# instadeepai/FrameDiPT

Hardware: AMD Instinct MI355X
Metric: residue*diffusion-steps/sec (higher is better)
Workload: dtype fp16

## Files before the change

### framedipt_amd/csrc/rowblock.hip

```cpp
#include <type_traits>

#include "common.hpp"
#include "kernels.hpp"

#pragma clang fp contract(off)

#define RB_SROW 144

typedef fd_h rb_hx4 __attribute__((ext_vector_type(4)));
__device__ __forceinline__ hx8 rb_ld(const char* p) { return __builtin_bit_cast(hx8, *(const u16x8*)p); }
__host__ __device__ constexpr int rb_max(int a, int b) { return a > b ? a : b; }

template <int N, class F>
__device__ __forceinline__ void ch_rb_for(F&& f) {
  if constexpr (N > 0) {
    ch_rb_for<N - 1>(f);
    f(std::integral_constant<int, N - 1>{});
  }
}

template <int K0, int N1, int N2, int NOUT, int FLAGS>
struct RBShape {
  static constexpr int KS0 = (K0 + 15) / 16;
  static constexpr int NL = 1 + (N1 > 0) + (N2 > 0);
// ... 413 lines not shown
    w_load(std::integral_constant<int, 0>{}, (const char*)img, wave);
    if constexpr (SPLIT) w_load(std::integral_constant<int, 1>{}, (const char*)img_lo, wave);
  };
  auto put4 = [&](char* buf, int off, float v0, float v1, float v2, float v3) {
    const float v[4] = {v0, v1, v2, v3};
    rb_hx4 pk, pl;
#pragma unroll
    for (int q = 0; q < 4; ++q) {
      pk[q] = (fd_h)v[q];
      pl[q] = (fd_h)(v[q] - (float)pk[q]);
    }
    *(rb_hx4*)(buf + off) = pk;
    if constexpr (SPLIT) *(rb_hx4*)(buf + XLO + off) = pl;
  };
  w_first(a.wo, a.wol);
  {
    f32x4 xv[10];
#pragma unroll
    for (int k = 0; k < 10; ++k) {
      const int idx = tid + k * FD_THREADS, r = idx / 80, c4 = idx % 80;
      const int gr = row0 + r < a.M ? row0 + r : a.M - 1;
      xv[k] = *(const f32x4*)(a.att + (long)gr * a.ld + 4 * c4);
    }
    {
      constexpr int NC = 7 * TL_D + (POST ? TL_NP : 0), NCV = (NC + FD_THREADS - 1) / FD_THREADS;
      float cv[NCV];
#pragma unroll
      for (int k = 0; k < NCV; ++k) {
        const int v = tid + k * FD_THREADS, which = v / TL_D, c = v % TL_D;
        const float* src = which == 0 ? a.bo : which == 1 ? a.g1 : which == 2 ? a.be1 : which == 3 ? a.b1 : which == 4 ? a.b2 : which == 5 ? a.g2 : a.be2;
        cv[k] = v < 7 * TL_D ? src[c] : (POST && v < NC ? a.bp[v - 7 * TL_D] : 0.f);
      }
#pragma unroll
      for (int k = 0; k < NCV; ++k)
        if (tid + k * FD_THREADS < NC) cst[tid + k * FD_THREADS] = cv[k];
    }
#pragma unroll
    for (int k = 0; k < 10; ++k) {
      const int idx = tid + k * FD_THREADS, r = idx / 80, c4 = idx % 80;
      put4(xs, r * TL_XROW + 8 * c4, xv[k][0], xv[k][1], xv[k][2], xv[k][3]);
    }
  }
  f32x4 rv[3][4];
#pragma unroll
  for (int u = 0; u < 3; ++u)
#pragma unroll
    for (int it = 0; it < 4; ++it) {
      const int T = wave + 4 * u < TL_NT ? wave + 4 * u : wave;
      const int r = 8 * it + (lane >> 3), gr = row0 + r < a.M ? row0 + r : a.M - 1;
      rv[u][it] = *(const f32x4*)(a.x + (long)gr * a.ld + 32 * T + 4 * (lane & 7));
    }
  f32x4 rvp[POST ? 2 : 1][4];
  auto load_rvp = [&]() {
#pragma unroll
    for (int u = 0; u < (POST ? 2 : 0); ++u)
#pragma unroll
      for (int it = 0; it < 4; ++it) {
        const int r = 8 * it + (lane >> 3), gr = row0 + r < a.M ? row0 + r : a.M - 1;
        rvp[u][it] = *(const f32x4*)(a.pres + (long)gr * a.ld_pres + 32 * (wave + 4 * u) + 4 * (lane & 7));
      }
  };
  if constexpr (POST && !SPLIT) load_rvp();
  const unsigned warm_tok = fd_l2_warm(a.warm, blockIdx.x, gridDim.x, tid, FD_THREADS);
  __syncthreads();
  FD_STAMP(1);
  hx8 X[TL_KS];
  f32x16 acc[3], xa[3];
  const char* xl_base = nullptr;
  auto x_load = [&](const char* buf) {
#pragma unroll
    for (int s = 0; s < TL_KS; ++s) X[s] = rb_ld(buf + li * TL_XROW + 32 * s + 16 * hi);
    xl_base = buf + XLO + li * TL_XROW + 16 * hi;
  };
  auto layer = [&](const void* img_, const void* img_lo_, auto NTC) {
    constexpr int NT = decltype(NTC)::value, NU = (NT + 3) / 4;
    const char* img = (const char*)img_;
    const char* img_lo = (const char*)img_lo_;
    ch_rb_for<NU>([&](auto U) {
      constexpr int u = decltype(U)::value;
      const int T = wave + 4 * u;
      const bool more = u + 1 < NU && T + 4 < NT;
      if constexpr (SPLIT) {
        constexpr int HB = (2 * u) % 3, LB = (2 * u + 1) % 3, FB = (2 * u + 2) % 3;
        if (more) w_load(std::integral_constant<int, FB>{}, img, T + 4);
        if (T < NT) {
          f32x16 c;
#pragma unroll
          for (int r = 0; r < 16; ++r) c[r] = 0.f;
#pragma unroll
          for (int s = 0; s < TL_KS; ++s) c = fd_mfma32(Wf[HB][s], X[s], c);
          {
            hx8 xr[3];
            xr[0] = rb_ld(xl_base);
            xr[1] = rb_ld(xl_base + 32);
            __builtin_amdgcn_sched_barrier(0);
#pragma unroll
            for (int s = 0; s < TL_KS; ++s) {
              if (s + 2 < TL_KS) xr[(s + 2) % 3] = rb_ld(xl_base + 32 * (s + 2));
              c = fd_mfma32(Wf[HB][s], xr[s % 3], c);
              __builtin_amdgcn_sched_barrier(0);
            }
          }
          if (more) w_load(std::integral_constant<int, HB>{}, img_lo, T + 4);
#pragma unroll
          for (int s = 0; s < TL_KS; ++s) c = fd_mfma32(Wf[LB][s], X[s], c);
          acc[u] = c;
        }
      } else {
        if (more) {
          if (u & 1) w_load(std::integral_constant<int, 0>{}, img, T + 4);
          else w_load(std::integral_constant<int, 1>{}, img, T + 4);
        }
        if (T < NT) {
          f32x16 c;
#pragma unroll
          for (int r = 0; r < 16; ++r) c[r] = 0.f;
#pragma unroll
          for (int s = 0; s < TL_KS; ++s) c = fd_mfma32(Wf[u & 1][s], X[s], c);
          acc[u] = c;
        }
      }
    });
  };
  constexpr std::integral_constant<int, TL_NT> NT_D{};
  auto layernorm = [&](const float* gam, const float* bet) {
    float s1 = 0.f, s2 = 0.f;
#pragma unroll
    for (int u = 0; u < 3; ++u)
      if (wave + 4 * u < TL_NT)
#pragma unroll
        for (int r = 0; r < 16; ++r) {
          s1 += acc[u][r];
          s2 += acc[u][r] * acc[u][r];
        }
    s1 += __shfl_xor(s1, 32, 64);
    s2 += __shfl_xor(s2, 32, 64);
    __syncthreads();
    if (hi == 0) {
      red[0][wave][li] = s1;
      red[1][wave][li] = s2;
    }
    __syncthreads();
    const float mu = (red[0][0][li] + red[0][1][li] + red[0][2][li] + red[0][3][li]) * (1.0f / TL_D);
    const float ex2 = (red[1][0][li] + red[1][1][li] + red[1][2][li] + red[1][3][li]) * (1.0f / TL_D);
    const float rstd = 1.0f / sqrtf(fmaxf(ex2 - mu * mu, 0.f) + 1e-5f);
#pragma unroll
    for (int u = 0; u < 3; ++u) {
      const int T = wave + 4 * u;
      if (T < TL_NT)
#pragma unroll
        for (int g = 0; g < 4; ++g) {
          const int f0 = 32 * T + 8 * g + 4 * hi;
          const f32x4 gm = *(const f32x4*)(gam + f0), bt = *(const f32x4*)(bet + f0);
#pragma unroll
          for (int q = 0; q < 4; ++q) acc[u][4 * g + q] = (acc[u][4 * g + q] - mu) * rstd * gm[q] + bt[q];
        }
    }
  };
  x_load(xs);
  layer(a.wo, a.wol, NT_D);
  FD_STAMP(2);
  w_first(a.w1, a.w1l);
#pragma unroll
  for (int u = 0; u < 3; ++u) {
    const int T = wave + 4 * u;
    if (T < TL_NT) {
#pragma unroll
      for (int it = 0; it < 4; ++it) *(f32x4*)(stg + (8 * it + (lane >> 3)) * RB_SROW + 16 * (lane & 7)) = rv[u][it];
#pragma unroll
      for (int g = 0; g < 4; ++g) {
        const f32x4 bv = *(const f32x4*)(cst + 32 * T + 8 * g + 4 * hi);
        const f32x4 rr = *(const f32x4*)(stg + li * RB_SROW + (8 * g + 4 * hi) * 4);
#pragma unroll
        for (int q = 0; q < 4; ++q) acc[u][4 * g + q] += bv[q] + rr[q];
      }
    }
  }
  layernorm(cst + TL_D, cst + 2 * TL_D);
  FD_STAMP(3);
#pragma unroll
  for (int u = 0; u < 3; ++u) {
    const int T = wave + 4 * u;
    xa[u] = acc[u];
    if (T < TL_NT)
#pragma unroll
      for (int g = 0; g < 4; ++g) {
        const int f0 = 32 * T + 8 * g + 4 * hi;
        put4(hs, li * TL_XROW + 2 * f0, acc[u][4 * g], acc[u][4 * g + 1], acc[u][4 * g + 2], acc[u][4 * g + 3]);
      }
  }
  __syncthreads();
  x_load(hs);
  FD_STAMP(4);
  layer(a.w1, a.w1l, NT_D);
  FD_STAMP(5);
  w_first(a.w2, a.w2l);
#pragma unroll
  for (int u = 0; u < 3; ++u) {
    const int T = wave + 4 * u;
    if (T < TL_NT)
#pragma unroll
      for (int g = 0; g < 4; ++g) {
        const int f0 = 32 * T + 8 * g + 4 * hi;
        const f32x4 bv = *(const f32x4*)(cst + 3 * TL_D + f0);
        put4(xs, li * TL_XROW + 2 * f0, fmaxf(acc[u][4 * g] + bv[0], 0.f), fmaxf(acc[u][4 * g + 1] + bv[1], 0.f),
             fmaxf(acc[u][4 * g + 2] + bv[2], 0.f), fmaxf(acc[u][4 * g + 3] + bv[3], 0.f));
      }
  }
  __syncthreads();
  x_load(xs);
  FD_STAMP(6);
  layer(a.w2, a.w2l, NT_D);
  FD_STAMP(7);
#pragma unroll
  for (int u = 0; u < 3; ++u) {
    const int T = wave + 4 * u;
    if (T < TL_NT)
#pragma unroll
      for (int g = 0; g < 4; ++g) {
        const f32x4 bv = *(const f32x4*)(cst + 4 * TL_D + 32 * T + 8 * g + 4 * hi);
#pragma unroll
        for (int q = 0; q < 4; ++q) acc[u][4 * g + q] += bv[q] + xa[u][4 * g + q];
      }
  }
  if constexpr (POST && SPLIT) load_rvp();
  if constexpr (POST) w_first(a.wp, a.wpl);
  layernorm(cst + 5 * TL_D, cst + 6 * TL_D);
  FD_STAMP(8);
  if constexpr (POST) {
#pragma unroll
    for (int u = 0; u < 3; ++u) {
      const int T = wave + 4 * u;
      if (T < TL_NT)
#pragma unroll
        for (int g = 0; g < 4; ++g) {
          const int f0 = 32 * T + 8 * g + 4 * hi;
          put4(hs, li * TL_XROW + 2 * f0, acc[u][4 * g], acc[u][4 * g + 1], acc[u][4 * g + 2], acc[u][4 * g + 3]);
        }
    }
    __syncthreads();
    x_load(hs);
    layer(a.wp, a.wpl, std::integral_constant<int, TL_NP / 32>{});
#pragma unroll
    for (int u = 0; u < 2; ++u) {
      const int T = wave + 4 * u;
#pragma unroll
      for (int it = 0; it < 4; ++it) *(f32x4*)(stg + (8 * it + (lane >> 3)) * RB_SROW + 16 * (lane & 7)) = rvp[u][it];
#pragma unroll
      for (int g = 0; g < 4; ++g) {
        const f32x4 bv = *(const f32x4*)(cst + 7 * TL_D + 32 * T + 8 * g + 4 * hi);
        const f32x4 rr = *(const f32x4*)(stg + li * RB_SROW + (8 * g + 4 * hi) * 4);
        f32x4 o;
#pragma unroll
        for (int q = 0; q < 4; ++q) o[q] = acc[u][4 * g + q] + bv[q] + rr[q];
        *(f32x4*)(stg + li * RB_SROW + (8 * g + 4 * hi) * 4) = o;
      }
#pragma unroll
      for (int it = 0; it < 4; ++it) {
        const int r = 8 * it + (lane >> 3);
        const f32x4 o = *(const f32x4*)(stg + r * RB_SROW + 16 * (lane & 7));
        if (row0 + r < a.M) *(f32x4*)(a.pout + (long)(row0 + r) * a.ld_pout + 32 * T + 4 * (lane & 7)) = o;
      }
    }
    fd_l2_warm_done(warm_tok);
    return;
  }
#pragma unroll
  for (int u = 0; u < 3; ++u) {
    const int T = wave + 4 * u;
    if (T < TL_NT) {
#pragma unroll
      for (int g = 0; g < 4; ++g) {
        f32x4 o = {acc[u][4 * g], acc[u][4 * g + 1], acc[u][4 * g + 2], acc[u][4 * g + 3]};
        *(f32x4*)(stg + li * RB_SROW + (8 * g + 4 * hi) * 4) = o;
      }
#pragma unroll
      for (int it = 0; it < 4; ++it) {
        const int r = 8 * it + (lane >> 3);
        const f32x4 o = *(const f32x4*)(stg + r * RB_SROW + 16 * (lane & 7));
        if (row0 + r < a.M) *(f32x4*)(a.out + (long)(row0 + r) * a.ld + 32 * T + 4 * (lane & 7)) = o;
      }
    }
  }
  fd_l2_warm_done(warm_tok);
}

#define RB16_BLOCKS 1
#define T16_KS (TL_D / 32)
#define T16_NT (TL_D / 16)
#define T16_XROW (TL_D * 2 + 32)
#define T16_XLO (16 * T16_XROW)
#define T16_SMEM (4 * T16_XLO + (7 * TL_D + TL_NP) * 4 + 2 * 4 * 16 * 4 + 16)
template <bool POST>
__global__ __launch_bounds__(FD_THREADS, RB16_BLOCKS) void tfmr_tail16_kernel(TfmrTailArgs a) {
  extern __shared__ __attribute__((aligned(16))) char smem[];
  char* xs = smem;
  char* hs = xs + 2 * T16_XLO;
  float* cst = (float*)(hs + 2 * T16_XLO);
  float (*red)[4][16] = (float (*)[4][16])(cst + 7 * TL_D + TL_NP);
  const int tid = threadIdx.x, lane = tid & 63, wave = tid >> 6, lr = lane & 15, fg = lane >> 4;
  const int row0 = blockIdx.x * 16;
  const long grow = row0 + lr < a.M ? row0 + lr : a.M - 1;
  FD_STAMP(0);
  hx8 Wh[2][T16_KS], Wl[2][T16_KS];
  auto w_load = [&](auto BUF, const void* img, const void* img_lo, int T) {
    constexpr int b = decltype(BUF)::value;
#pragma unroll
    for (int s = 0; s < T16_KS; ++s) {
      Wh[b][s] = rb_ld((const char*)img + ((size_t)(T * T16_KS + s) * 64 + lane) * 16);
      Wl[b][s] = rb_ld((const char*)img_lo + ((size_t)(T * T16_KS + s) * 64 + lane) * 16);
    }
  };
  auto put4 = [&](char* buf, int off, float v0, float v1, float v2, float v3) {
    const float v[4] = {v0, v1, v2, v3};
    rb_hx4 pk, pl;
#pragma unroll
    for (int q = 0; q < 4; ++q) {
      pk[q] = (fd_h)v[q];
      pl[q] = (fd_h)(v[q] - (float)pk[q]);
    }
    *(rb_hx4*)(buf + off) = pk;
    *(rb_hx4*)(buf + T16_XLO + off) = pl;
  };
  constexpr std::integral_constant<int, 0> B0{};
  constexpr std::integral_constant<int, 1> B1{};
  w_load(B0, a.wo, a.wol, wave);
  {
    f32x4 xv[5];
#pragma unroll
    for (int k = 0; k < 5; ++k) {
      const int idx = tid + k * FD_THREADS, r = idx / 80, c4 = idx % 80;
      const int gr = row0 + r < a.M ? row0 + r : a.M - 1;
      xv[k] = *(const f32x4*)(a.att + (long)gr * a.ld + 4 * c4);
    }
    {
      constexpr int NC = 7 * TL_D + (POST ? TL_NP : 0), NCV = (NC + FD_THREADS - 1) / FD_THREADS;
      float cv[NCV];
#pragma unroll
      for (int k = 0; k < NCV; ++k) {
        const int v = tid + k * FD_THREADS, which = v / TL_D, c = v % TL_D;
        const float* src = which == 0 ? a.bo : which == 1 ? a.g1 : which == 2 ? a.be1 : which == 3 ? a.b1 : which == 4 ? a.b2 : which == 5 ? a.g2 : a.be2;
        cv[k] = v < 7 * TL_D ? src[c] : (POST && v < NC ? a.bp[v - 7 * TL_D] : 0.f);
      }
#pragma unroll
      for (int k = 0; k < NCV; ++k)
        if (tid + k * FD_THREADS < NC) cst[tid + k * FD_THREADS] = cv[k];
    }
#pragma unroll
    for (int k = 0; k < 5; ++k) {
      const int idx = tid + k * FD_THREADS, r = idx / 80, c4 = idx % 80;
      put4(xs, r * T16_XROW + 8 * c4, xv[k][0], xv[k][1], xv[k][2], xv[k][3]);
    }
  }
  f32x4 rv[5];
#pragma unroll
  for (int u = 0; u < 5; ++u) rv[u] = *(const f32x4*)(a.x + grow * a.ld + 16 * (wave + 4 * u) + 4 * fg);
  const unsigned warm_tok = fd_l2_warm(a.warm, blockIdx.x, gridDim.x, tid, FD_THREADS);
  __syncthreads();
  FD_STAMP(1);
  hx8 X[T16_KS];
  const char* xl_base = nullptr;
  auto x_load = [&](const char* buf) {
#pragma unroll
    for (int s = 0; s < T16_KS; ++s) X[s] = rb_ld(buf + lr * T16_XROW + (32 * s + 8 * fg) * 2);
    xl_base = buf + T16_XLO + lr * T16_XROW + 16 * fg;
  };
  f32x4 acc[5], xa[5];
  auto mma = [](hx8 w, hx8 x, f32x4 c) {
    return fd_mfma16(w, x, c);
  };
  auto layer = [&](const void* img, const void* img_lo, auto NTC) {
    constexpr int NT = decltype(NTC)::value, NU = NT / 4;
    ch_rb_for<NU>([&](auto U) {
      constexpr int u = decltype(U)::value, b = u & 1;
      const int T = wave + 4 * u;
      if constexpr (u + 1 < NU) {
        if constexpr (b == 0) w_load(B1, img, img_lo, T + 4);
        else w_load(B0, img, img_lo, T + 4);
      }
      f32x4 c = {0.f, 0.f, 0.f, 0.f};
#pragma unroll
      for (int s = 0; s < T16_KS; ++s) c = mma(Wh[b][s], X[s], c);
      {
        hx8 xr[3];
        xr[0] = rb_ld(xl_base);
        xr[1] = rb_ld(xl_base + 64);
#pragma unroll
        for (int s = 0; s < T16_KS; ++s) {
          if (s + 2 < T16_KS) xr[(s + 2) % 3] = rb_ld(xl_base + 64 * (s + 2));
          c = mma(Wh[b][s], xr[s % 3], c);
        }
      }
#pragma unroll
      for (int s = 0; s < T16_KS; ++s) c = mma(Wl[b][s], X[s], c);
      acc[u] = c;
      asm volatile("s_waitcnt lgkmcnt(0)" ::: "memory");
    });
  };
  constexpr std::integral_constant<int, T16_NT> NT_D{};
  auto layernorm = [&](const float* gam, const float* bet) {
    float s1 = 0.f, s2 = 0.f;
#pragma unroll
    for (int u = 0; u < 5; ++u)
#pragma unroll
      for (int i = 0; i < 4; ++i) {
        s1 += acc[u][i];
        s2 += acc[u][i] * acc[u][i];
      }
    s1 += __shfl_xor(s1, 16, 64); s2 += __shfl_xor(s2, 16, 64);
    s1 += __shfl_xor(s1, 32, 64); s2 += __shfl_xor(s2, 32, 64);
    __syncthreads();
    if (fg == 0) {
      red[0][wave][lr] = s1;
      red[1][wave][lr] = s2;
    }
    __syncthreads();
    const float mu = (red[0][0][lr] + red[0][1][lr] + red[0][2][lr] + red[0][3][lr]) * (1.0f / TL_D);
    const float ex2 = (red[1][0][lr] + red[1][1][lr] + red[1][2][lr] + red[1][3][lr]) * (1.0f / TL_D);
    const float rstd = 1.0f / sqrtf(fmaxf(ex2 - mu * mu, 0.f) + 1e-5f);
#pragma unroll
    for (int u = 0; u < 5; ++u) {
      const int f0 = 16 * (wave + 4 * u) + 4 * fg;
      const f32x4 gm = *(const f32x4*)(gam + f0), bt = *(const f32x4*)(bet + f0);
#pragma unroll
      for (int i = 0; i < 4; ++i) acc[u][i] = (acc[u][i] - mu) * rstd * gm[i] + bt[i];
    }
  };
  x_load(xs);
  layer(a.wo, a.wol, NT_D);
  FD_STAMP(2);
  w_load(B0, a.w1, a.w1l, wave);
#pragma unroll
  for (int u = 0; u < 5; ++u) {
    const f32x4 bv = *(const f32x4*)(cst + 16 * (wave + 4 * u) + 4 * fg);
#pragma unroll
    for (int i = 0; i < 4; ++i) acc[u][i] += bv[i] + rv[u][i];
  }
  layernorm(cst + TL_D, cst + 2 * TL_D);
  FD_STAMP(3);
#pragma unroll
  for (int u = 0; u < 5; ++u) {
    xa[u] = acc[u];
    put4(hs, lr * T16_XROW + 2 * (16 * (wave + 4 * u) + 4 * fg), acc[u][0], acc[u][1], acc[u][2], acc[u][3]);
  }
  __syncthreads();
  x_load(hs);
  FD_STAMP(4);
  layer(a.w1, a.w1l, NT_D);
  FD_STAMP(5);
  w_load(B0, a.w2, a.w2l, wave);
#pragma unroll
  for (int u = 0; u < 5; ++u) {
    const int f0 = 16 * (wave + 4 * u) + 4 * fg;
    const f32x4 bv = *(const f32x4*)(cst + 3 * TL_D + f0);
    put4(xs, lr * T16_XROW + 2 * f0, fmaxf(acc[u][0] + bv[0], 0.f), fmaxf(acc[u][1] + bv[1], 0.f), fmaxf(acc[u][2] + bv[2], 0.f),
         fmaxf(acc[u][3] + bv[3], 0.f));
  }
  __syncthreads();
  x_load(xs);
  FD_STAMP(6);
  layer(a.w2, a.w2l, NT_D);
  FD_STAMP(7);
#pragma unroll
  for (int u = 0; u < 5; ++u) {
    const f32x4 bv = *(const f32x4*)(cst + 4 * TL_D + 16 * (wave + 4 * u) + 4 * fg);
#pragma unroll
    for (int i = 0; i < 4; ++i) acc[u][i] += bv[i] + xa[u][i];
  }
  f32x4 rvp[4];
  if constexpr (POST) {
    w_load(B0, a.wp, a.wpl, wave);
  }
  layernorm(cst + 5 * TL_D, cst + 6 * TL_D);
  FD_STAMP(8);
  if constexpr (POST) {
#pragma unroll
    for (int u = 0; u < 5; ++u)
      put4(hs, lr * T16_XROW + 2 * (16 * (wave + 4 * u) + 4 * fg), acc[u][0], acc[u][1], acc[u][2], acc[u][3]);
    __syncthreads();
    x_load(hs);
#pragma unroll
    for (int u = 0; u < 4; ++u) rvp[u] = *(const f32x4*)(a.pres + grow * a.ld_pres + 16 * (wave + 4 * u) + 4 * fg);
    layer(a.wp, a.wpl, std::integral_constant<int, TL_NP / 16>{});
#pragma unroll
    for (int u = 0; u < 4; ++u) {
      const int f0 = 16 * (wave + 4 * u) + 4 * fg;
      const f32x4 bv = *(const f32x4*)(cst + 7 * TL_D + f0);
      f32x4 o;
#pragma unroll
      for (int i = 0; i < 4; ++i) o[i] = acc[u][i] + bv[i] + rvp[u][i];
      if (row0 + lr < a.M) *(f32x4*)(a.pout + (long)(row0 + lr) * a.ld_pout + f0) = o;
    }
    fd_l2_warm_done(warm_tok);
    return;
  }
#pragma unroll
  for (int u = 0; u < 5; ++u)
    if (row0 + lr < a.M) *(f32x4*)(a.out + (long)(row0 + lr) * a.ld + 16 * (wave + 4 * u) + 4 * fg) = acc[u];
  fd_l2_warm_done(warm_tok);
}

#define TR_D 256
#define TR_KS (TR_D / 32)
#define TR_NT (TR_D / 16)
#define TR_XROW (TR_D * 2 + 32)
#define TR_XLO (16 * TR_XROW)
#define TR_NC (11 * TR_D)
#define TR_SMEM (4 * TR_XLO + TR_NC * 4 + 2 * 4 * 16 * 4 + 4 * 16 * 8 * 4 + 64 + 16)
template <int KS0, int NL, bool LN, bool BB, bool SKIP = false, bool ETR = false>
__global__ __launch_bounds__(FD_THREADS, RB16_BLOCKS) void mlp16_kernel(RowBlockArgs a, int k0) {
  extern __shared__ __attribute__((aligned(16))) char smem[];
  char* xs = smem;
  char* hs = xs + 2 * TR_XLO;
  float* cst = (float*)(hs + 2 * TR_XLO);
  float (*red)[4][16] = (float (*)[4][16])(cst + TR_NC);
  float* red3 = (float*)(red + 2);
  float* pmask = red3 + 4 * 16 * 8;
  const int tid = threadIdx.x, lane = tid & 63, wave = tid >> 6, lr = lane & 15, fg = lane >> 4;
  const int row0 = blockIdx.x * 16;
  const long grow = row0 + lr < a.M ? row0 + lr : a.M - 1;
  hx8 Wh[2][TR_KS], Wl[2][TR_KS];
  auto w_load = [&](auto BUF, auto KSC, const void* img, const void* img_lo, int T) {
    constexpr int b = decltype(BUF)::value, KS = decltype(KSC)::value;
#pragma unroll
    for (int s = 0; s < KS; ++s) {
      Wh[b][s] = rb_ld((const char*)img + ((size_t)(T * KS + s) * 64 + lane) * 16);
      Wl[b][s] = rb_ld((const char*)img_lo + ((size_t)(T * KS + s) * 64 + lane) * 16);
    }
  };
  constexpr std::integral_constant<int, KS0> K0C{};
  constexpr std::integral_constant<int, TR_KS> K8C{};
  auto put4 = [&](char* buf, int off, float v0, float v1, float v2, float v3) {
    const float v[4] = {v0, v1, v2, v3};
    rb_hx4 pk, pl;
#pragma unroll
    for (int q = 0; q < 4; ++q) {
      pk[q] = (fd_h)v[q];
      pl[q] = (fd_h)(v[q] - (float)pk[q]);
    }
    *(rb_hx4*)(buf + off) = pk;
    *(rb_hx4*)(buf + TR_XLO + off) = pl;
  };
  constexpr std::integral_constant<int, 0> B0{};
  constexpr std::integral_constant<int, 1> B1{};
  w_load(B0, K0C, a.w0, a.w0l, wave);
  {
    constexpr int C4 = KS0 * 8, NV = (16 * C4 + FD_THREADS - 1) / FD_THREADS;
    f32x4 xv[NV];
#pragma unroll
    for (int k = 0; k < NV; ++k) {
      const int idx = tid + k * FD_THREADS, r = idx / C4, c4 = idx % C4;
      const int gr = row0 + r < a.M ? row0 + r : a.M - 1;
      xv[k] = f32x4{0.f, 0.f, 0.f, 0.f};
      if (idx < 16 * C4 && 4 * c4 < k0) xv[k] = *(const f32x4*)(a.in + (long)gr * a.ld_in + 4 * c4);
    }
    {
      constexpr int NCV = TR_NC / FD_THREADS;
      float cv[NCV];
#pragma unroll
      for (int k = 0; k < NCV; ++k) {
        const int v = tid + k * FD_THREADS, which = v / TR_D, c = v % TR_D;
        cv[k] = which == 0 ? a.b0[c] : which == 1 ? a.b1[c] : which == 2 ? (NL == 3 ? a.b2[c] : 0.f) : which == 3 ? (LN ? a.gamma[c] : 1.f)
                : which == 4 ? (LN ? a.beta[c] : 0.f) : (BB ? a.bb_w[v - 5 * TR_D] : 0.f);
      }
#pragma unroll
      for (int k = 0; k < NCV; ++k) cst[tid + k * FD_THREADS] = cv[k];
    }
    if (tid < 16) pmask[tid] = a.rowmask_post ? a.rowmask_post[row0 + tid < a.M ? row0 + tid : a.M - 1] : 1.f;
#pragma unroll
    for (int k = 0; k < NV; ++k) {
      const int idx = tid + k * FD_THREADS, r = idx / C4, c4 = idx % C4;
      if (idx < 16 * C4) put4(xs, r * TR_XROW + 8 * c4, xv[k][0], xv[k][1], xv[k][2], xv[k][3]);
    }
  }
  f32x4 rv[4];
#pragma unroll
  for (int u = 0; u < 4; ++u) {
    rv[u] = f32x4{0.f, 0.f, 0.f, 0.f};
    if (a.residual) rv[u] = *(const f32x4*)(a.residual + grow * a.ld_res + 16 * (wave + 4 * u) + 4 * fg);
  }
  const unsigned warm_tok = fd_l2_warm(a.warm, blockIdx.x, gridDim.x, tid, FD_THREADS);
  __syncthreads();
  hx8 X[TR_KS];
  const char* xl_base = nullptr;
  auto x_load = [&](auto KSC, const char* buf) {
#pragma unroll
    for (int s = 0; s < decltype(KSC)::value; ++s) X[s] = rb_ld(buf + lr * TR_XROW + (32 * s + 8 * fg) * 2);
    xl_base = buf + TR_XLO + lr * TR_XROW + 16 * fg;
  };
  f32x4 acc[4];
  auto mma = [](hx8 w, hx8 x, f32x4 c) {
    return fd_mfma16(w, x, c);
  };
  auto layer = [&](auto KSC, const void* img, const void* img_lo) {
    constexpr int KS = decltype(KSC)::value;
    ch_rb_for<4>([&](auto U) {
      constexpr int u = decltype(U)::value, b = u & 1;
      const int T = wave + 4 * u;
      if constexpr (u + 1 < 4) {
        if constexpr (b == 0) w_load(B1, KSC, img, img_lo, T + 4);
        else w_load(B0, KSC, img, img_lo, T + 4);
      }
      f32x4 c = {0.f, 0.f, 0.f, 0.f};
#pragma unroll
      for (int s = 0; s < KS; ++s) c = mma(Wh[b][s], X[s], c);
      {
        hx8 xr[3];
        xr[0] = rb_ld(xl_base);
        if (KS > 1) xr[1] = rb_ld(xl_base + 64);
#pragma unroll
        for (int s = 0; s < KS; ++s) {
          if (s + 2 < KS) xr[(s + 2) % 3] = rb_ld(xl_base + 64 * (s + 2));
          c = mma(Wh[b][s], xr[s % 3], c);
        }
      }
#pragma unroll
      for (int s = 0; s < KS; ++s) c = mma(Wl[b][s], X[s], c);
      acc[u] = c;
    });
  };
  auto relu_to = [&](char* dst, const float* bias) {
#pragma unroll
    for (int u = 0; u < 4; ++u) {
      const int f0 = 16 * (wave + 4 * u) + 4 * fg;
      const f32x4 bv = *(const f32x4*)(bias + f0);
      put4(dst, lr * TR_XROW + 2 * f0, fmaxf(acc[u][0] + bv[0], 0.f), fmaxf(acc[u][1] + bv[1], 0.f), fmaxf(acc[u][2] + bv[2], 0.f),
           fmaxf(acc[u][3] + bv[3], 0.f));
    }
  };
  x_load(K0C, xs);
  layer(K0C, a.w0, a.w0l);
  w_load(B0, K8C, a.w1, a.w1l, wave);
  relu_to(hs, cst);
  __syncthreads();
  x_load(K8C, hs);
  layer(K8C, a.w1, a.w1l);
  if constexpr (NL == 3) {
    w_load(B0, K8C, a.w2, a.w2l, wave);
    relu_to(xs, cst + TR_D);
    __syncthreads();
    x_load(K8C, xs);
    layer(K8C, a.w2, a.w2l);
  }
  float s1 = 0.f, s2 = 0.f;
#pragma unroll
  for (int u = 0; u < 4; ++u) {
    const f32x4 bv = *(const f32x4*)(cst + (NL - 1) * TR_D + 16 * (wave + 4 * u) + 4 * fg);
#pragma unroll
    for (int i = 0; i < 4; ++i) {
      const float v = acc[u][i] + bv[i] + rv[u][i];
      acc[u][i] = v;
      s1 += v;
    }
  }
  float mu = 0.f, rstd = 1.f;
  if constexpr (LN) {
    s1 += __shfl_xor(s1, 16, 64); s1 += __shfl_xor(s1, 32, 64);
    if (fg == 0) red[0][wave][lr] = s1;
    __syncthreads();
    mu = (red[0][0][lr] + red[0][1][lr] + red[0][2][lr] + red[0][3][lr]) * (1.0f / TR_D);
#pragma unroll
    for (int u = 0; u < 4; ++u)
#pragma unroll
      for (int i = 0; i < 4; ++i) {
        const float dlt = acc[u][i] - mu;
        s2 += dlt * dlt;
      }
    s2 += __shfl_xor(s2, 16, 64); s2 += __shfl_xor(s2, 32, 64);
    if (fg == 0) red[1][wave][lr] = s2;
    __syncthreads();
    rstd = 1.0f / sqrtf((red[1][0][lr] + red[1][1][lr] + red[1][2][lr] + red[1][3][lr]) * (1.0f / TR_D) + 1e-5f);
  }
  const float pm = pmask[lr];
  float pd[6] = {0.f, 0.f, 0.f, 0.f, 0.f, 0.f};
#pragma unroll
  for (int u = 0; u < 4; ++u) {
    const int f0 = 16 * (wave + 4 * u) + 4 * fg;
    const f32x4 gm = *(const f32x4*)(cst + 3 * TR_D + f0), bt = *(const f32x4*)(cst + 4 * TR_D + f0);
    f32x4 o;
#pragma unroll
    for (int i = 0; i < 4; ++i) o[i] = LN ? ((acc[u][i] - mu) * rstd * gm[i] + bt[i]) * pm : acc[u][i] * pm;
    if (row0 + lr < a.M) *(f32x4*)(a.out + (long)(row0 + lr) * a.ld_out + f0) = o;
    if constexpr (BB) {
#pragma unroll
      for (int k = 0; k < 6; ++k) {
        const f32x4 wv = *(const f32x4*)(cst + 5 * TR_D + k * TR_D + f0);
        pd[k] += (o[0] * wv[0] + o[1] * wv[1]) + (o[2] * wv[2] + o[3] * wv[3]);
      }
    }
  }
  if constexpr (SKIP || ETR) {
    w_load(B0, K8C, SKIP ? a.w3 : a.we0, SKIP ? a.w3l : a.we0l, wave);
#pragma unroll
    for (int u = 0; u < 4; ++u) {
      const int f0 = 16 * (wave + 4 * u) + 4 * fg;
      const f32x4 gm = *(const f32x4*)(cst + 3 * TR_D + f0), bt = *(const f32x4*)(cst + 4 * TR_D + f0);
      put4(hs, lr * TR_XROW + 2 * f0, LN ? ((acc[u][0] - mu) * rstd * gm[0] + bt[0]) * pm : acc[u][0] * pm,
           LN ? ((acc[u][1] - mu) * rstd * gm[1] + bt[1]) * pm : acc[u][1] * pm, LN ? ((acc[u][2] - mu) * rstd * gm[2] + bt[2]) * pm : acc[u][2] * pm,
           LN ? ((acc[u][3] - mu) * rstd * gm[3] + bt[3]) * pm : acc[u][3] * pm);
    }
    __syncthreads();
    x_load(K8C, hs);
    if constexpr (SKIP) {
    layer(K8C, a.w3, a.w3l);
#pragma unroll
    for (int u = 0; u < 4; ++u) {
      const int f0 = 16 * (wave + 4 * u) + 4 * fg;
      const f32x4 bv = *(const f32x4*)(a.b3 + f0);
      f32x4 o;
#pragma unroll
      for (int i = 0; i < 4; ++i) o[i] = acc[u][i] + bv[i];
      if (row0 + lr < a.M) *(f32x4*)(a.out2 + (long)(row0 + lr) * a.ld_out2 + f0) = o;
    }
    }
  }
  if constexpr (ETR) {
    f32x4 ea[2];
    ch_rb_for<2>([&](auto U) {
      constexpr int u = decltype(U)::value;
      const int T = wave + 4 * u;
      if constexpr (u == 0) w_load(B1, K8C, a.we0, a.we0l, T + 4);
      f32x4 c = {0.f, 0.f, 0.f, 0.f};
#pragma unroll
      for (int s = 0; s < TR_KS; ++s) c = mma(Wh[u][s], X[s], c);
      {
        hx8 xr[3];
        xr[0] = rb_ld(xl_base);
        xr[1] = rb_ld(xl_base + 64);
#pragma unroll
        for (int s = 0; s < TR_KS; ++s) {
          if (s + 2 < TR_KS) xr[(s + 2) % 3] = rb_ld(xl_base + 64 * (s + 2));
          c = mma(Wh[u][s], xr[s % 3], c);
        }
      }
#pragma unroll
      for (int s = 0; s < TR_KS; ++s) c = mma(Wl[u][s], X[s], c);
      ea[u] = c;
    });
    constexpr std::integral_constant<int, 4> K4C{};
    auto e2_load = [&](auto J, int T) {
      constexpr int j = decltype(J)::value, b = j & 1, h = j >> 1;
#pragma unroll
      for (int s = 0; s < 4; ++s) {
        Wh[b][4 * h + s] = rb_ld((const char*)a.we1 + ((size_t)(T * 4 + s) * 64 + lane) * 16);
        Wl[b][4 * h + s] = rb_ld((const char*)a.we1l + ((size_t)(T * 4 + s) * 64 + lane) * 16);
      }
    };
    e2_load(std::integral_constant<int, 2>{}, wave);
    e2_load(std::integral_constant<int, 3>{}, wave + 4);
#pragma unroll
    for (int u = 0; u < 2; ++u) {
      const int f0 = 16 * (wave + 4 * u) + 4 * fg;
      const f32x4 bv = *(const f32x4*)(a.be0 + f0);
      put4(xs, lr * TR_XROW + 2 * f0, ea[u][0] + bv[0], ea[u][1] + bv[1], ea[u][2] + bv[2], ea[u][3] + bv[3]);
    }
    e2_load(std::integral_constant<int, 0>{}, wave + 8);
    __syncthreads();
    x_load(K4C, xs);
    const int NJ4 = a.img_N >> 2, r0 = row0 + 4 * fg;
    half_t* ia = (half_t*)a.img_a;
    half_t* ib = (half_t*)a.img_b;
    const int rb_ = r0 < a.M ? r0 / a.img_N : 0, jt_ = r0 < a.M ? (r0 - rb_ * a.img_N) >> 2 : 0;
    float bvs[16];
#pragma unroll
    for (int u = 0; u < 16; ++u) bvs[u] = a.be1[16 * (wave + 4 * u) + lr];
    ch_rb_for<16>([&](auto U) {
      constexpr int u = decltype(U)::value, j = (u + 2) & 3, b = j & 1, h = j >> 1;
      const int T = wave + 4 * u;
      if constexpr (u + 3 < 16) e2_load(std::integral_constant<int, (u + 5) & 3>{}, T + 12);
      f32x4 c = {0.f, 0.f, 0.f, 0.f};
#pragma unroll
      for (int s = 0; s < 4; ++s) c = mma(X[s], Wh[b][4 * h + s], c);
#pragma unroll
      for (int s = 0; s < 4; ++s) c = mma(rb_ld(xl_base + 64 * s), Wh[b][4 * h + s], c);
#pragma unroll
      for (int s = 0; s < 4; ++s) c = mma(X[s], Wl[b][4 * h + s], c);
      const float bv = bvs[u];
      const int T32 = T >> 1, f = 16 * (T & 1) + lr;
      u16x4 o = {0, 0, 0, 0};
      if (r0 < a.M) o = u16x4{f2h(c[0] + bv), f2h(c[1] + bv), f2h(c[2] + bv), f2h(c[3] + bv)};
      if (T32 < 16) {
        if ((r0 >> 3) < ((a.M + 7) >> 3)) *(u16x4*)(ia + ((((long)(r0 >> 3) * 16 + T32) * 32 + f) << 3) + (r0 & 4)) = o;
      } else if (r0 < a.M) {
        half_t* dst = ib + ((((long)rb_ * NJ4 + jt_) * 16 + (T32 - 16)) * 32 + f) * 8;
        *(u16x4*)dst = o;
        if (rb_ > 0) *(u16x4*)(dst - (long)NJ4 * 16 * 32 * 8 + 4) = o;
// ... 156 lines not shown
```

Baseline: 1.141 million.

## Prefetch transformer-tail weights two tiles ahead across layer boundaries

Replaces per-layer weight loading with a global tile counter spanning the wo, w1, w2 and wp layers. Each tile's weights are prefetched two steps ahead into a double buffer, and the hi and lo halves are loaded separately after the MFMA groups that consume them. The aim is to hide global-memory weight latency, including at layer transitions where loads were previously issued just before use. This adds register pressure and relies on the buffer index parity (g&1) staying consistent while loads are in flight.

After: 1.149 million (median of 6 runs). About the same (+0.7%).

```diff
diff --git a/framedipt_amd/csrc/rowblock.hip b/framedipt_amd/csrc/rowblock.hip
--- a/framedipt_amd/csrc/rowblock.hip
+++ b/framedipt_amd/csrc/rowblock.hip
@@ -739,15 +739,24 @@
   const int row0 = blockIdx.x * 16;
   const long grow = row0 + lr < a.M ? row0 + lr : a.M - 1;
   FD_STAMP(0);
+  constexpr int NG = 15 + (POST ? TL_NP / 64 : 0);
   hx8 Wh[2][T16_KS], Wl[2][T16_KS];
-  auto w_load = [&](auto BUF, const void* img, const void* img_lo, int T) {
-    constexpr int b = decltype(BUF)::value;
-#pragma unroll
-    for (int s = 0; s < T16_KS; ++s) {
-      Wh[b][s] = rb_ld((const char*)img + ((size_t)(T * T16_KS + s) * 64 + lane) * 16);
-      Wl[b][s] = rb_ld((const char*)img_lo + ((size_t)(T * T16_KS + s) * 64 + lane) * 16);
-    }
-  };
+  auto w_load = [&](auto GC, auto LOC) {
+    constexpr int g = decltype(GC)::value, k = g / 5, b = g & 1;
+    constexpr bool lo = decltype(LOC)::value;
+    if constexpr (g < NG) {
+      const char* img = (const char*)(k == 0 ? (lo ? a.wol : a.wo) : k == 1 ? (lo ? a.w1l : a.w1) : k == 2 ? (lo ? a.w2l : a.w2) : (lo ? a.wpl : a.wp));
+      const int T = wave + 4 * (g % 5);
+#pragma unroll
+      for (int s = 0; s < T16_KS; ++s) {
+        const hx8 v = rb_ld(img + ((size_t)(T * T16_KS + s) * 64 + lane) * 16);
+        if constexpr (lo) Wl[b][s] = v;
+        else Wh[b][s] = v;
+      }
+    }
+  };
+  constexpr std::integral_constant<bool, false> HI{};
+  constexpr std::integral_constant<bool, true> LO{};
   auto put4 = [&](char* buf, int off, float v0, float v1, float v2, float v3) {
     const float v[4] = {v0, v1, v2, v3};
     rb_hx4 pk, pl;
@@ -759,9 +768,6 @@
     *(rb_hx4*)(buf + off) = pk;
     *(rb_hx4*)(buf + T16_XLO + off) = pl;
   };
-  constexpr std::integral_constant<int, 0> B0{};
-  constexpr std::integral_constant<int, 1> B1{};
-  w_load(B0, a.wo, a.wol, wave);
   {
     f32x4 xv[5];
 #pragma unroll
@@ -779,6 +785,10 @@
         const float* src = which == 0 ? a.bo : which == 1 ? a.g1 : which == 2 ? a.be1 : which == 3 ? a.b1 : which == 4 ? a.b2 : which == 5 ? a.g2 : a.be2;
         cv[k] = v < 7 * TL_D ? src[c] : (POST && v < NC ? a.bp[v - 7 * TL_D] : 0.f);
       }
+      w_load(std::integral_constant<int, 0>{}, HI);
+      w_load(std::integral_constant<int, 0>{}, LO);
+      w_load(std::integral_constant<int, 1>{}, HI);
+      w_load(std::integral_constant<int, 1>{}, LO);
 #pragma unroll
       for (int k = 0; k < NCV; ++k)
         if (tid + k * FD_THREADS < NC) cst[tid + k * FD_THREADS] = cv[k];
@@ -806,15 +816,11 @@
   auto mma = [](hx8 w, hx8 x, f32x4 c) {
     return fd_mfma16(w, x, c);
   };
-  auto layer = [&](const void* img, const void* img_lo, auto NTC) {
-    constexpr int NT = decltype(NTC)::value, NU = NT / 4;
+  auto layer = [&](auto G0C, auto NUC) {
+    constexpr int G0 = decltype(G0C)::value, NU = decltype(NUC)::value;
     ch_rb_for<NU>([&](auto U) {
-      constexpr int u = decltype(U)::value, b = u & 1;
-      const int T = wave + 4 * u;
-      if constexpr (u + 1 < NU) {
-        if constexpr (b == 0) w_load(B1, img, img_lo, T + 4);
-        else w_load(B0, img, img_lo, T + 4);
-      }
+      constexpr int u = decltype(U)::value, g = G0 + u, b = g & 1;
+      constexpr std::integral_constant<int, g + 2> GN{};
       f32x4 c = {0.f, 0.f, 0.f, 0.f};
 #pragma unroll
       for (int s = 0; s < T16_KS; ++s) c = mma(Wh[b][s], X[s], c);
@@ -828,13 +834,15 @@
           c = mma(Wh[b][s], xr[s % 3], c);
         }
       }
+      w_load(GN, HI);
 #pragma unroll
       for (int s = 0; s < T16_KS; ++s) c = mma(Wl[b][s], X[s], c);
+      w_load(GN, LO);
       acc[u] = c;
       asm volatile("s_waitcnt lgkmcnt(0)" ::: "memory");
     });
   };
-  constexpr std::integral_constant<int, T16_NT> NT_D{};
+  constexpr std::integral_constant<int, T16_NT / 4> NU_D{};
   auto layernorm = [&](const float* gam, const float* bet) {
     float s1 = 0.f, s2 = 0.f;
 #pragma unroll
@@ -864,9 +872,8 @@
     }
   };
   x_load(xs);
-  layer(a.wo, a.wol, NT_D);
+  layer(std::integral_constant<int, 0>{}, NU_D);
   FD_STAMP(2);
-  w_load(B0, a.w1, a.w1l, wave);
 #pragma unroll
   for (int u = 0; u < 5; ++u) {
     const f32x4 bv = *(const f32x4*)(cst + 16 * (wave + 4 * u) + 4 * fg);
@@ -883,9 +890,8 @@
   __syncthreads();
   x_load(hs);
   FD_STAMP(4);
-  layer(a.w1, a.w1l, NT_D);
+  layer(std::integral_constant<int, 5>{}, NU_D);
   FD_STAMP(5);
-  w_load(B0, a.w2, a.w2l, wave);
 #pragma unroll
   for (int u = 0; u < 5; ++u) {
     const int f0 = 16 * (wave + 4 * u) + 4 * fg;
@@ -896,7 +902,7 @@
   __syncthreads();
   x_load(xs);
   FD_STAMP(6);
-  layer(a.w2, a.w2l, NT_D);
+  layer(std::integral_constant<int, 10>{}, NU_D);
   FD_STAMP(7);
 #pragma unroll
   for (int u = 0; u < 5; ++u) {
@@ -905,9 +911,6 @@
     for (int i = 0; i < 4; ++i) acc[u][i] += bv[i] + xa[u][i];
   }
   f32x4 rvp[4];
-  if constexpr (POST) {
-    w_load(B0, a.wp, a.wpl, wave);
-  }
   layernorm(cst + 5 * TL_D, cst + 6 * TL_D);
   FD_STAMP(8);
   if constexpr (POST) {
@@ -918,7 +921,7 @@
     x_load(hs);
 #pragma unroll
     for (int u = 0; u < 4; ++u) rvp[u] = *(const f32x4*)(a.pres + grow * a.ld_pres + 16 * (wave + 4 * u) + 4 * fg);
-    layer(a.wp, a.wpl, std::integral_constant<int, TL_NP / 16>{});
+    layer(std::integral_constant<int, 15>{}, std::integral_constant<int, TL_NP / 64>{});
 #pragma unroll
     for (int u = 0; u < 4; ++u) {
       const int f0 = 16 * (wave + 4 * u) + 4 * fg;
```
